# ylsung/vl-merging

Hardware: AMD Instinct MI355X
Metric: VL samples/sec (fwd+bwd) base_vl 384^2 at 1/2/4/8 GPUs; merge GB/s vs HBM peak (higher is better)
Workload: dtype bf16

## Files before the change

include/vlm_hip.h:

```cpp
#ifndef VLM_HIP_H
#define VLM_HIP_H
#include <stddef.h>
#include <stdint.h>

#ifdef __cplusplus
extern "C" {
#endif

#define VLM_OK 0
#define VLM_ERR_ARG (-1)
#define VLM_ERR_LAUNCH (-2)
#define VLM_ERR_WORKSPACE (-3)
#define VLM_ERR_UNSUPPORTED (-4)

#define VLM_ABI_VERSION 11
int vlm_abi_version(void);
int vlm_device_cus(void);
int vlm_set_cu_budget(int cus);
int vlm_debug_occupy(int workgroups, int threads, int lds_bytes, int microseconds, void* stream);

#define VLM_MERGE_LERP 0
#define VLM_MERGE_TASKVEC 1
#define VLM_MERGE_MEAN 2
#define VLM_MERGE_MAX_SRC 4
// ... 392 lines not shown
                  int ldc, int c_is_f32, const vlm_epilogue_t* epi, void* stream);
int vlm_gemm_bf16_live(int ta, int tb, int M, int N, int K, const void* A, int lda, const void* B, int ldb, void* C,
                       int ldc, int c_is_f32, const vlm_epilogue_t* epi, const float* row_live, void* stream);
#define VLM_GEMM_MAX_GROUPS 4
typedef struct {
  int32_t row0, rows;
  const void* B;
  int32_t ldb;
  int32_t reserved;
  const float* bias;
  float* col_sum;
  float* col_sum_ws;
} vlm_gemm_group_t;
int vlm_gemm_bf16_grouped(int n_groups, const vlm_gemm_group_t* groups, int N, int K, const void* A, int lda, void* C,
                          int ldc, int c_is_f32, const vlm_epilogue_t* epi, void* stream);
typedef struct {
  int32_t row0, rows;
  float* C;
  int32_t accumulate;
  int32_t reserved;
} vlm_wgrad_group_t;
int vlm_gemm_wgrad_grouped(int n_groups, const vlm_wgrad_group_t* groups, int M, int N, const void* A, int lda,
                           const void* B, int ldb, int ldc, float* splitk_ws, uint64_t splitk_ws_bytes, void* stream);
typedef struct {
  const void* dy;
  int32_t ld_dy, M;
  const void* x;
  int32_t ld_x, N;
  float* dW;
  int32_t ldc, accumulate;
} vlm_wgrad_problem_t;
int vlm_gemm_wgrad_batch(int n, const vlm_wgrad_problem_t* problems, int T, float* splitk_ws, uint64_t splitk_ws_bytes,
                         void* stream);
int vlm_gemm_set_big_tile_mode(int mode);

int vlm_layernorm_fwd(const float* x, int ldx, int M, int D, const float* gamma, const float* beta, float eps,
                      void* y, int ldy, int y_is_f32, float* stats, void* stream);
#define VLM_ROW_WS_BYTES(D) ((size_t)1536 * 2 * (size_t)(D) * sizeof(float))
int vlm_layernorm_bwd(const void* dy, int lddy, int dy_is_f32, const float* x, int ldx, const float* stats,
                      const float* gamma, int M, int D, const float* dres, int lddres, float* dx, int lddx,
                      float* dgamma, float* dbeta, float* workspace, size_t workspace_bytes, int* deferred_blocks,
                      void* stream);
typedef struct {
  const void* y;
  int32_t ldy;
  const float* gamma;
  const float* row_scale;
  void* dy;
  int32_t lddy;
  float* dgamma;
  float* dbias;
  float* workspace;
  size_t workspace_bytes;
} vlm_layerscale_t;
int vlm_layernorm_bwd_scale(const void* dy, int lddy, int dy_is_f32, const float* x, int ldx, const float* stats,
                            const float* gamma, int M, int D, const float* dres, int lddres, float* dx, int lddx,
                            float* dgamma, float* dbeta, float* workspace, size_t workspace_bytes,
                            const vlm_layerscale_t* scale, int* deferred_blocks, void* stream);
#define VLM_MAX_FOLD_JOBS 16
typedef struct {
  const float* partials;
  int32_t nblocks;
  int32_t D;
  float* out0;
  float* out1;
} vlm_fold_job_t;
// ... 188 lines not shown
```

vl-merging_amd/_lib.py:

```python
import ctypes
import os

_HERE = os.path.dirname(os.path.abspath(__file__))
LIB_PATH = os.environ.get("VLM_LIB_PATH") or os.path.join(_HERE, "lib", "libvlm_hip.so")
_lib = None

c_void_p = ctypes.c_void_p
c_int = ctypes.c_int
c_float = ctypes.c_float
c_size_t = ctypes.c_size_t
c_u64 = ctypes.c_uint64

MERGE_LERP, MERGE_TASKVEC, MERGE_MEAN = 0, 1, 2
MERGE_MAX_SRC = 4


class MergeJob(ctypes.Structure):
    _fields_ = [
        ("dst", c_void_p),
        ("base", c_void_p),
        ("src", c_void_p * MERGE_MAX_SRC),
        ("ratio", c_float * MERGE_MAX_SRC),
        ("n_src", ctypes.c_int32),
        ("mode", ctypes.c_int32),
# ... 370 lines not shown
    "vlm_band_plan_bytes": (c_size_t, [c_int, c_u64]),
    "vlm_band_plan_upload": (c_int, [ctypes.POINTER(BandJob), c_int, c_void_p, c_size_t, c_void_p]),
    "vlm_band_run": (c_int, [c_void_p, c_void_p]),
    "vlm_della_plan_bytes": (c_size_t, [c_int, c_u64]),
    "vlm_della_plan_upload": (c_int, [ctypes.POINTER(DellaJob), c_int, c_void_p, c_size_t, c_void_p]),
    "vlm_della_run": (c_int, [c_void_p, c_void_p]),
    "vlm_pairstats_plan_bytes": (c_size_t, [c_int, c_u64]),
    "vlm_pairstats_plan_upload": (c_int, [ctypes.POINTER(PairStatsJob), c_int, c_void_p, c_size_t, c_void_p]),
    "vlm_pairstats_run": (c_int, [c_void_p, c_void_p]),
    "vlm_stock_plan_bytes": (c_size_t, [c_int, c_u64]),
    "vlm_stock_plan_upload": (c_int, [ctypes.POINTER(StockJob), c_int, c_void_p, c_size_t, c_void_p]),
    "vlm_stock_run": (c_int, [c_void_p, c_void_p]),
    "vlm_sce_plan_bytes": (c_size_t, [c_int, c_u64]),
    "vlm_sce_plan_upload": (c_int, [ctypes.POINTER(SceJob), c_int, c_void_p, c_size_t, c_void_p]),
    "vlm_sce_run": (c_int, [c_void_p, c_void_p]),
    "vlm_sphere_plan_bytes": (c_size_t, [c_int, c_u64]),
    "vlm_sphere_plan_upload": (c_int, [ctypes.POINTER(SphereJob), c_int, c_void_p, c_size_t, c_void_p]),
    "vlm_sphere_run": (c_int, [c_void_p, c_void_p]),
    "vlm_tall_plan_bytes": (c_size_t, [c_int, c_u64]),
    "vlm_tall_plan_upload": (c_int, [ctypes.POINTER(TallJob), c_int, c_void_p, c_size_t, c_void_p]),
    "vlm_tall_run": (c_int, [c_void_p, c_void_p]),
    "vlm_emr_plan_bytes": (c_size_t, [c_int, c_u64]),
    "vlm_emr_plan_upload": (c_int, [ctypes.POINTER(EmrJob), c_int, c_void_p, c_size_t, c_void_p]),
    "vlm_emr_run": (c_int, [c_void_p, c_void_p]),
    "vlm_gemm_bf16": (c_int, [c_int, c_int, c_int, c_int, c_int, c_void_p, c_int, c_void_p, c_int, c_void_p, c_int,
                              c_int, ctypes.POINTER(Epilogue), c_void_p]),
    "vlm_gemm_bf16_live": (c_int, [c_int, c_int, c_int, c_int, c_int, c_void_p, c_int, c_void_p, c_int, c_void_p, c_int,
                                   c_int, ctypes.POINTER(Epilogue), c_void_p, c_void_p]),
    "vlm_gemm_bf16_grouped": (c_int, [c_int, ctypes.POINTER(GemmGroup), c_int, c_int, c_void_p, c_int, c_void_p, c_int, c_int,
                                      ctypes.POINTER(Epilogue), c_void_p]),
    "vlm_gemm_wgrad_grouped": (c_int, [c_int, ctypes.POINTER(WgradGroup), c_int, c_int, c_void_p, c_int, c_void_p, c_int, c_int,
                                       c_void_p, c_u64, c_void_p]),
    "vlm_gemm_wgrad_batch": (c_int, [c_int, ctypes.POINTER(WgradProblem), c_int, c_void_p, c_u64, c_void_p]),
    "vlm_attention_fwd": (c_int, [ctypes.POINTER(AttnDesc), c_void_p, c_int, c_void_p, c_void_p]),
    "vlm_attention_bwd_ws_floats": (c_size_t, [ctypes.POINTER(AttnDesc), c_int]),
    "vlm_attention_qkeep_served": (c_int, [ctypes.POINTER(AttnDesc), c_int]),
    "vlm_attention_bwd": (c_int, [ctypes.POINTER(AttnDesc), c_void_p, c_int, c_void_p, c_int, c_void_p, c_void_p, c_size_t,
                                  c_void_p, c_int, c_void_p, c_void_p, c_void_p]),
    "vlm_attention_bwd_live": (c_int, [ctypes.POINTER(AttnDesc), c_void_p, c_int, c_void_p, c_int, c_void_p, c_void_p, c_size_t,
                                       c_void_p, c_int, c_void_p, c_void_p, c_void_p, c_void_p]),
    "vlm_layernorm_fwd": (c_int, [c_void_p, c_int, c_int, c_int, c_void_p, c_void_p, c_float, c_void_p, c_int, c_int,
                                  c_void_p, c_void_p]),
    "vlm_layernorm_bwd": (c_int, [c_void_p, c_int, c_int, c_void_p, c_int, c_void_p, c_void_p, c_int, c_int, c_void_p,
                                  c_int, c_void_p, c_int, c_void_p, c_void_p, c_void_p, c_size_t,
                                  ctypes.POINTER(c_int), c_void_p]),
    "vlm_layernorm_bwd_scale": (c_int, [c_void_p, c_int, c_int, c_void_p, c_int, c_void_p, c_void_p, c_int, c_int, c_void_p,
                                        c_int, c_void_p, c_int, c_void_p, c_void_p, c_void_p, c_size_t,
                                        ctypes.POINTER(LayerScale), ctypes.POINTER(c_int), c_void_p]),
    "vlm_layerscale_bwd": (c_int, [c_void_p, c_int, c_void_p, c_int, c_void_p, c_void_p, c_int, c_int, c_void_p, c_int,
                                   c_void_p, c_void_p, c_void_p, c_size_t, ctypes.POINTER(c_int), c_void_p]),
    "vlm_colreduce_batch": (c_int, [ctypes.POINTER(FoldJob), c_int, c_void_p]),
    "vlm_gemm_set_big_tile_mode": (c_int, [c_int]),
    "vlm_colsum_bf16": (c_int, [c_void_p, c_int, c_int, c_int, c_void_p, c_void_p]),
    "vlm_adamw_step": (c_int, [c_void_p, c_void_p, c_void_p, c_void_p, c_void_p, c_u64, c_float, c_float, c_float,
                               c_float, c_float, c_float, c_float, c_int, c_void_p]),
    "vlm_accumulate_f32_f64": (c_int, [c_void_p, c_void_p, c_u64, c_void_p]),
    "vlm_gram_f64": (c_int, [c_void_p, c_int, c_int, c_int, c_int, c_void_p, c_void_p]),
    "vlm_gemm_f64": (c_int, [c_int, c_int, c_int, c_int, c_int, ctypes.c_double, c_void_p, c_int, c_int, c_void_p, c_int,
                             ctypes.c_double, c_void_p, c_int, c_void_p]),
    "vlm_scale_gram_f64": (c_int, [c_void_p, c_void_p, c_int, ctypes.c_double, c_int, c_void_p]),
    "vlm_cholesky_f64": (c_int, [c_void_p, c_int, c_void_p, c_void_p]),
    "vlm_solve_spd_right_f64": (c_int, [c_void_p, c_int, c_void_p, c_int, c_int, c_void_p]),
    "vlm_gemm_f64_batched": (c_int, [c_int, c_int, c_int, c_int, c_int, ctypes.c_double, ctypes.POINTER(c_void_p), c_int, c_int,
                                     ctypes.POINTER(c_void_p), c_int, ctypes.c_double, ctypes.POINTER(c_void_p), c_int, c_int, c_void_p]),
    "vlm_cholesky_f64_batched": (c_int, [ctypes.POINTER(c_void_p), c_int, c_int, c_void_p, c_void_p]),
    "vlm_solve_spd_right_f64_batched": (c_int, [ctypes.POINTER(c_void_p), c_int, ctypes.POINTER(c_void_p), c_int, c_int, c_int, c_void_p]),
# ... 103 lines not shown
```

vl-merging_amd/csrc/gemm.hip:

```cpp
#include "vlm_common.h"
#include "vlm_diag.h"
#include "wgrad_plan.h"
#include <atomic>

#define GEMM_BM 128
#define GEMM_BN 128
#define GEMM_BK 64
#define GEMM_THREADS 256
#define GEMM_TILE_BYTES (GEMM_BM * GEMM_BK * 2)

typedef __attribute__((address_space(3))) s16x4 lds_s16x4;

__device__ __forceinline__ float gelu_cdf(float x, float& ez2) {
  const float t = __builtin_amdgcn_rcpf(fmaf(0.3275911f * 0.70710678118654752440f, fabsf(x), 1.0f));
  ez2 = __builtin_amdgcn_exp2f((x * x) * (-0.5f * 1.4426950408889634f));
  float poly = fmaf(t, 0.5f * 1.061405429f, 0.5f * -1.453152027f);
  poly = fmaf(t, poly, 0.5f * 1.421413741f);
  poly = fmaf(t, poly, 0.5f * -0.284496736f);
  poly = fmaf(t, poly, 0.5f * 0.254829592f);
  const float e = fmaf(-(poly * t), ez2, 0.5f);
  return 0.5f + copysignf(e, x);
}
__device__ __forceinline__ float gelu_erf(float x) {
  float ez2;
// ... 910 lines not shown
  asm volatile("s_waitcnt lgkmcnt(0)" ::: "memory");
  __builtin_amdgcn_s_barrier();
  BIG_READ(fa0, fb0, sA0, sB0)
  GEMM_STAMP(1)

  int kt = 0;
  for (; kt < nk - 4; kt += 2) {
    BIG_STEP(kt + 0, 1, 1, 1, fa0, fb0, fa1, fb1, ra0, rb0, sA0, sB0, sA1, sB1)
    BIG_STEP(kt + 1, 1, 1, 1, fa1, fb1, fa0, fb0, ra1, rb1, sA1, sB1, sA0, sB0)
  }
#define BIG_TAIL_STEPS()                                                               \
  BIG_STEP(kt + 0, 0, 1, 1, fa0, fb0, fa1, fb1, ra0, rb0, sA0, sB0, sA1, sB1)          \
  BIG_STEP(kt + 1, 0, 1, 1, fa1, fb1, fa0, fb0, ra1, rb1, sA1, sB1, sA0, sB0)          \
  BIG_STEP(kt + 2, 0, 0, 1, fa0, fb0, fa1, fb1, ra0, rb0, sA0, sB0, sA1, sB1)          \
  BIG_STEP(kt + 3, 0, 0, 0, fa1, fb1, fa0, fb0, ra1, rb1, sA1, sB1, sA0, sB0)
  if constexpr (DEEP) {
    BIG_TAIL_STEPS()
    GEMM_STAMP(2)
    big_epilogue_t<OUT_F32, RES, AUX> ep(p, wl, mw0, nw0, lane);
    float* ws_row = (p.epi.col_sum_ws && mw0 + 128 <= (uint32_t)p.M) ? p.epi.col_sum_ws + ((size_t)(tm_ws * 2 + wm) * 2) * p.N : nullptr;
    BIG_EPILOGUE_LOOP_DEEP(AHEAD)
    ep.finish(lane, ws_row);
  } else {
    EPIL_SETUP()
    BIG_TAIL_STEPS()
    GEMM_STAMP(2)
    float* ws_row = (p.epi.col_sum_ws && mw0 + 128 <= (uint32_t)p.M) ? p.epi.col_sum_ws + ((size_t)(tm_ws * 2 + wm) * 2) * p.N : nullptr;
    BIG_EPILOGUE_LOOP()
    ep.finish(lane, ws_row);
  }
  GEMM_STAMP_END()
}

template <bool GROUPED = false>
__global__ __launch_bounds__(GEMM_THREADS, 1) void vlm_gemm_bigT_kernel(const gemm_params_t p) {
  __shared__ __attribute__((aligned(1024))) unsigned char sA0[BIG_OP_BYTES], sA1[BIG_OP_BYTES], sB0[BIG_OP_BYTES], sB1[BIG_OP_BYTES];
  __shared__ __attribute__((aligned(16))) unsigned char epl[4 * EPIL_WAVE_BYTES];
  const int tid = threadIdx.x;
  const int lane = tid & 63;
  const int wave = __builtin_amdgcn_readfirstlane(tid >> 6);
  const int wm = wave >> 1, wn = wave & 1;
  uint32_t ntile = p.tiles_m * p.tiles_n, tiles_n = (uint32_t)p.tiles_n;
  const uint32_t q8 = gridDim.x >> 3, r8 = gridDim.x & 7, xcd = blockIdx.x & 7;
  uint32_t item = (xcd < r8 ? xcd * (q8 + 1) : r8 * (q8 + 1) + (xcd - r8) * q8) + (blockIdx.x >> 3);
  uint32_t k_base = 0, k_end = (uint32_t)p.K, ws_base = 0;
  int nk = p.ksteps_per_split;
  const void *A = p.A, *B = p.B;
  uint32_t lda = (uint32_t)p.lda, ldb = (uint32_t)p.ldb;
  int M = p.M, N = p.N;
  if constexpr (GROUPED) {
    int g = 0;
#pragma unroll
    for (int i = 1; i < VLM_GEMM_MAX_GROUPS; ++i)
      if (i < p.n_groups && item >= (uint32_t)p.grpT[i].item0) g = i;
    const gemmT_group_t G = p.grpT[g];
    item -= (uint32_t)G.item0;
    k_base = (uint32_t)G.row0;
    k_end = (uint32_t)G.row_end;
    nk = G.kps;
    ws_base = G.ws_base;
    A = G.A; B = G.B;
    lda = (uint32_t)G.lda; ldb = (uint32_t)G.ldb;
    M = G.M; N = G.N;
    ntile = (uint32_t)G.ntile; tiles_n = (uint32_t)G.tiles_n;
  }
  const uint32_t split = item / ntile, tile = item - split * ntile;
  const uint32_t tm = tile / tiles_n, tn = tile - tm * tiles_n;
  const uint32_t m0 = tm * BIG_BM, n0 = tn * BIG_BN;
  const uint32_t k_first = k_base + split * (uint32_t)nk * BIG_BK;
  const __amdgpu_buffer_rsrc_t ra =
      __builtin_amdgcn_make_buffer_rsrc(const_cast<void*>(A), 0, (int)((uint64_t)k_end * lda * 2), 0x00020000);
  const __amdgpu_buffer_rsrc_t rb =
      __builtin_amdgcn_make_buffer_rsrc(const_cast<void*>(B), 0, (int)((uint64_t)k_end * ldb * 2), 0x00020000);

  uint32_t offa[4], offb[4], wr_off[4];
#pragma unroll
  for (int u = 0; u < 4; ++u) {
    const uint32_t row = 2 * (wave + 4 * u) + (lane >> 5), c16 = lane & 31;
    offa[u] = ((k_first + row) * lda + m0 + c16 * 8) * 2;
    offb[u] = ((k_first + row) * ldb + n0 + c16 * 8) * 2;
    wr_off[u] = row * 512 + (((c16 >> 1) ^ ((row & 3) | (((row >> 3) & 1) << 2))) << 5) + (c16 & 1) * 16;
  }
  uint32_t rda[8], rdb[8];
  {
// ... 48 lines not shown
    BIG_MFMA(FCA, FCB)                                                                   \
    _Pragma("unroll") for (int g = 0; g < 32; ++g) {                                     \
      __builtin_amdgcn_sched_group_barrier(0x008, 1, 0);                                 \
      __builtin_amdgcn_sched_group_barrier(0x100, 1, 0);                                 \
    }                                                                                    \
    _Pragma("unroll") for (int g = 0; g < 8; ++g) {                                      \
      __builtin_amdgcn_sched_group_barrier(0x008, 2, 0);                                 \
      __builtin_amdgcn_sched_group_barrier(0x200, 1, 0);                                 \
      __builtin_amdgcn_sched_group_barrier(0x008, 2, 0);                                 \
      __builtin_amdgcn_sched_group_barrier(0x020, 1, 0);                                 \
    }                                                                                    \
    __builtin_amdgcn_sched_barrier(0);                                                   \
  }
  BIGT_GLOAD(ra0, rb0, 0)
  BIGT_GLOAD(ra1, rb1, 1)
  BIGT_LWRITE(ra0, rb0, sA0, sB0)
  BIGT_GLOAD(ra0, rb0, 2)
  BIGT_LWRITE(ra1, rb1, sA1, sB1)
  BIGT_GLOAD(ra1, rb1, 3)
  asm volatile("s_waitcnt lgkmcnt(0)" ::: "memory");
  __builtin_amdgcn_s_barrier();
  BIGT_READ(fa0, fb0, sA0, sB0)
  int kt = 0;
  for (; kt < nk - 4; kt += 2) {
    BIGT_STEP(kt + 0, 1, 1, 1, fa0, fb0, fa1, fb1, ra0, rb0, sA0, sB0, sA1, sB1)
    BIGT_STEP(kt + 1, 1, 1, 1, fa1, fb1, fa0, fb0, ra1, rb1, sA1, sB1, sA0, sB0)
  }
  BIGT_STEP(kt + 0, 0, 1, 1, fa0, fb0, fa1, fb1, ra0, rb0, sA0, sB0, sA1, sB1)
  BIGT_STEP(kt + 1, 0, 1, 1, fa1, fb1, fa0, fb0, ra1, rb1, sA1, sB1, sA0, sB0)
  BIGT_STEP(kt + 2, 0, 0, 1, fa0, fb0, fa1, fb1, ra0, rb0, sA0, sB0, sA1, sB1)
  BIGT_STEP(kt + 3, 0, 0, 0, fa1, fb1, fa0, fb0, ra1, rb1, sA1, sB1, sA0, sB0)

  gemm_params_t pl = p;
  pl.C = reinterpret_cast<float*>(p.C) + ws_base + (size_t)split * M * N;
  pl.M = M;
  pl.N = N;
  pl.ldc = N;
  const uint32_t mw0 = m0 + wm * 128, nw0 = n0 + wn * 128;
  unsigned char* const wl = epl + wave * EPIL_WAVE_BYTES;
  big_epilogue_t<true, false, 0, 128, 0, true> ep(pl, wl, mw0, nw0, lane);
  epil_in_t inA, inB;
  ep.load_inputs(inA, 0);
  BIG_EPILOGUE_LOOP()
}

__global__ __launch_bounds__(256) void splitk_reduce_kernel(const float* __restrict__ ws, int splits, int M, int N, float* __restrict__ C,
                                                            int ldc, int accumulate) {
  const size_t i = (size_t)blockIdx.x * 256 + threadIdx.x, per = (size_t)M * N / 4;
  if (i >= per) return;
  const size_t e = i * 4, m = e / N, n = e - m * N;
  f32x4 t = accumulate ? *reinterpret_cast<const f32x4*>(C + m * ldc + n) : (f32x4){0.f, 0.f, 0.f, 0.f};
  for (int s = 0; s < splits; ++s) t += *reinterpret_cast<const f32x4*>(ws + (size_t)s * M * N + e);
  *reinterpret_cast<f32x4*>(C + m * ldc + n) = t;
}

struct splitk_groups_t {
  float* C[VLM_GEMM_MAX_GROUPS];
  int M[VLM_GEMM_MAX_GROUPS], N[VLM_GEMM_MAX_GROUPS], ldc[VLM_GEMM_MAX_GROUPS];
  uint32_t ws_base[VLM_GEMM_MAX_GROUPS];
  int splits[VLM_GEMM_MAX_GROUPS], accumulate[VLM_GEMM_MAX_GROUPS];
};
__global__ __launch_bounds__(256) void splitk_reduce_grouped_kernel(const float* __restrict__ ws, const splitk_groups_t g) {
  const int gi = blockIdx.y;
  const int N = g.N[gi], ldc = g.ldc[gi];
  const size_t i = (size_t)blockIdx.x * 256 + threadIdx.x, mn = (size_t)g.M[gi] * N;
  if (i >= mn / 4) return;
  float* const C = g.C[gi];
  const float* const w = ws + g.ws_base[gi];
  const size_t e = i * 4, m = e / N, n = e - m * N;
  f32x4 t = g.accumulate[gi] ? *reinterpret_cast<const f32x4*>(C + m * ldc + n) : (f32x4){0.f, 0.f, 0.f, 0.f};
  for (int s = 0; s < g.splits[gi]; ++s) t += *reinterpret_cast<const f32x4*>(w + (size_t)s * mn + e);
  *reinterpret_cast<f32x4*>(C + m * ldc + n) = t;
}

static int plan_cus() {
  const int cus = vlm_device_cus();
// ... 269 lines not shown
  p.n_groups = n;
  splitk_groups_t rg{};
  size_t per = 0;
  for (int g = 0; g < n; ++g) {
    const wgradT_problem_t& P = pr[g];
    const wgrad_plan_group_t& G = plan.g[g];
    p.grpT[g] = gemmT_group_t{P.A, P.B, P.lda, P.ldb, P.M, P.N, P.N / BIG_BN, in[g].tiles, P.row0, P.row_end, G.item0, G.kps,
                              (uint32_t)G.ws_base};
    rg.C[g] = P.C; rg.M[g] = P.M; rg.N[g] = P.N; rg.ldc[g] = P.ldc;
    rg.ws_base[g] = (uint32_t)G.ws_base; rg.splits[g] = G.splits; rg.accumulate[g] = P.accumulate;
    if ((size_t)P.M * P.N / 4 > per) per = (size_t)P.M * P.N / 4;
  }
  hipLaunchKernelGGL(vlm_gemm_bigT_kernel<true>, dim3(plan.items), dim3(GEMM_THREADS), 0, s, p);
  VLM_CHECK_LAUNCH();
  hipLaunchKernelGGL(splitk_reduce_grouped_kernel, dim3((unsigned)((per + 255) / 256), n), dim3(256), 0, s,
                     reinterpret_cast<const float*>(splitk_ws), rg);
  VLM_CHECK_LAUNCH();
  return VLM_OK;
}

extern "C" int vlm_gemm_wgrad_batch(int n, const vlm_wgrad_problem_t* problems, int T, float* splitk_ws, uint64_t splitk_ws_bytes,
                                    void* stream) {
  if (n < 1 || n > VLM_GEMM_MAX_GROUPS || !problems || T < 1) return VLM_ERR_ARG;
  wgradT_problem_t pr[VLM_GEMM_MAX_GROUPS];
  for (int i = 0; i < n; ++i) {
    const vlm_wgrad_problem_t& P = problems[i];
    if (!P.dy || !P.x || !P.dW || P.M < 1 || P.N < 1) return VLM_ERR_ARG;
    pr[i] = wgradT_problem_t{P.dy, P.x, P.ld_dy, P.ld_x, P.M, P.N, 0, T, P.dW, P.ldc, P.accumulate};
  }
  if (gemm_big_mode() <= 0) return 1;
  return launch_gemm_bigT_grouped(n, pr, splitk_ws, splitk_ws_bytes, (hipStream_t)stream);
}

extern "C" int vlm_gemm_wgrad_grouped(int n_groups, const vlm_wgrad_group_t* groups, int M, int N, const void* A, int lda,
                                      const void* B, int ldb, int ldc, float* splitk_ws, uint64_t splitk_ws_bytes, void* stream) {
  if (n_groups < 1 || n_groups > VLM_GEMM_MAX_GROUPS || !groups || M < 0 || N < 0) return VLM_ERR_ARG;
  int prev_end = 0;
  for (int g = 0; g < n_groups; ++g) {
    if (groups[g].row0 < prev_end || groups[g].rows < 0 || !groups[g].C) return VLM_ERR_ARG;
    prev_end = groups[g].row0 + groups[g].rows;
  }
  if (M == 0 || N == 0) return VLM_OK;
  if (!A || !B || (lda & 7) || (ldb & 7) || ((uintptr_t)A & 15) || ((uintptr_t)B & 15)) return VLM_ERR_ARG;
  hipStream_t s = (hipStream_t)stream;
  for (int g = 0; g < n_groups; ++g)
    if (groups[g].rows == 0 && !groups[g].accumulate &&
        hipMemset2DAsync(groups[g].C, (size_t)ldc * 4, 0, (size_t)N * 4, M, s) != hipSuccess)
      return VLM_ERR_LAUNCH;
  const int K_total = prev_end;
  if (gemm_big_mode() > 0 && (uint64_t)K_total * lda * 2 < (1ull << 31) && (uint64_t)K_total * ldb * 2 < (1ull << 31)) {
    wgradT_problem_t pr[VLM_GEMM_MAX_GROUPS];
    int live = 0;
    for (int g = 0; g < n_groups; ++g) {
      const vlm_wgrad_group_t& G = groups[g];
      if (G.rows > 0) pr[live++] = wgradT_problem_t{A, B, lda, ldb, M, N, G.row0, G.row0 + G.rows, G.C, ldc, G.accumulate};
    }
    if (live == 0) return VLM_OK;
    const int rc = launch_gemm_bigT_grouped(live, pr, splitk_ws, splitk_ws_bytes, s);
    if (rc <= 0) return rc;
  }
  for (int g = 0; g < n_groups; ++g) {
    const vlm_wgrad_group_t& G = groups[g];
    if (G.rows == 0) continue;
    vlm_epilogue_t e{};
    e.alpha = 1.0f;
    e.accumulate = G.accumulate;
// ... 11 lines not shown
```

vl-merging_amd/csrc/wgrad_plan.h:

```cpp
#pragma once
#include <stddef.h>
#include <stdint.h>

#define WGRAD_PLAN_MAX_GROUPS 4
#define WGRAD_PLAN_MIN_STEPS 16

struct wgrad_plan_in_t {
  int tiles;
  int ksteps;
  uint64_t mn;
};

struct wgrad_plan_group_t {
  int kps, splits;
  int item0;
  int slice0;
  uint64_t ws_base;
};

struct wgrad_plan_t {
  wgrad_plan_group_t g[WGRAD_PLAN_MAX_GROUPS];
  int items;
  int slices;
  uint64_t ws_floats;
// ... 7 lines not shown
    if (in[g].tiles == 0 || in[g].ksteps == 0) continue;
    tiles += in[g].tiles;
    work += (long)in[g].ksteps * in[g].tiles;
  }
  if (tiles == 0 || tiles > cus) return 1;
  long target = (work + cus - 1) / cus;
  if (target < WGRAD_PLAN_MIN_STEPS) target = WGRAD_PLAN_MIN_STEPS;
  for (;; target += 2) {
    long items = 0;
    for (int g = 0; g < n; ++g)
      if (in[g].tiles > 0 && in[g].ksteps > 0) items += ((in[g].ksteps + target - 1) / target) * in[g].tiles;
    if (items <= cus) break;
  }
  out->items = out->slices = 0;
  out->ws_floats = 0;
  for (int g = 0; g < n; ++g) {
    wgrad_plan_group_t& G = out->g[g];
    G = wgrad_plan_group_t{0, 0, out->items, out->slices, out->ws_floats};
    if (in[g].tiles == 0 || in[g].ksteps == 0) continue;
    const int nk = in[g].ksteps;
    int splits = (int)((nk + target - 1) / target);
    int kps = (nk + splits - 1) / splits;
    kps += kps & 1;
    if (kps < 4) kps = 4;
    splits = (nk + kps - 1) / kps;
    G.kps = kps;
    G.splits = splits;
    out->items += splits * in[g].tiles;
    out->slices += splits;
    out->ws_floats += (uint64_t)splits * in[g].mn;
  }
  return out->ws_floats > ws_floats ? 1 : 0;
}
```

vl-merging_amd/engine.py:

```python
import itertools
import math
import os
import weakref
from typing import List, Optional

import torch

from . import _lib as L
from . import ops

BF16, F32 = torch.bfloat16, torch.float32
ALIGN = 64


def _touch_hook(p):
    p._vlm_flat.touched.add(p._vlm_name)


def touch(*params):
    for p in params:
        if p is not None:
            f = getattr(p, "_vlm_flat", None)
            if f is not None:
                f.touched.add(p._vlm_name)
# ... 131 lines not shown
        layers = sorted(pend) if layer is None else ([layer] if layer in pend else [])
        if not layers:
            return
        jobs = [j for i in layers for j in self._ls_jobs.get(i, ())]
        side = wgrad_stream()
        if side is None:
            ops.layerscale_finish(jobs)
        else:
            side.wait_stream(torch.cuda.current_stream())
            with torch.cuda.stream(side):
                ops.layerscale_finish(jobs)
            if not _WGRAD["pending"]:
                torch.cuda.current_stream().wait_stream(side)
        for i in layers:
            pend.discard(i)

    def zero_grad(self):
        self.flat_g.zero_()
        if getattr(self, "ls_pending", None) or getattr(self, "_ls_armed", False):
            for jobs in getattr(self, "_ls_jobs", {}).values():
                for j in jobs:
                    j["raw_w"].zero_()
                    if j["raw_b"] is not None:
                        j["raw_b"].zero_()
            self.ls_pending.clear()
            self._ls_armed = False

    def slice_of(self, names):
        lo = min(self.offsets[n][0] for n in names)
        hi = max(self.offsets[n][0] + self.extent[n] for n in names)
        return lo, hi


_WGRAD = {"stream": None, "enabled": os.environ.get("VLM_WGRAD_STREAM", "1") != "0", "pending": False}


def wgrad_stream():
    if not _WGRAD["enabled"]:
        return None
    if _WGRAD["stream"] is None:
        _WGRAD["stream"] = torch.cuda.Stream()
    return _WGRAD["stream"]


def sync_wgrad():
    if _WGRAD["stream"] is not None:
        torch.cuda.current_stream().wait_stream(_WGRAD["stream"])
    _WGRAD["pending"] = False


def _arm_wgrad_join():
    if not _WGRAD["pending"]:
        _WGRAD["pending"] = True
        torch.autograd.Variable._execution_engine.queue_callback(sync_wgrad)


class _Side:

    def __init__(self, *tensors):
        self.s = wgrad_stream()
        self.tensors = tensors
        self.ctx = None

    def __enter__(self):
        if self.s is None:
            return self
        self.s.wait_stream(torch.cuda.current_stream())
# ... 508 lines not shown
        plan, pc = ctx.plan, ctx.pc
        x, st1, ln1, qkv, o, lse, y1, x1, st2, ln2, h, a, y2, rs1, rs2, bias_t, ok = ctx.saved_tensors
        kr = ctx.kr
        rs1 = rs1 if rs1.numel() else None
        rs2 = rs2 if rs2.numel() else None
        live_all = _live(rs1, plan, pc)
        if kr is not None:
            rs1, rs2 = kr.take(rs1), kr.take(rs2)
        live1, live2 = _live(rs1, plan, pc), _live(rs2, plan, pc)
        bias_t = bias_t if ctx.has_bias else None
        M_all, D = x.shape
        M = x1.shape[0]
        dev = x.device
        H = pc.H
        Fdim = h.shape[1]
        if ctx.kr_out is not None:
            dx2 = ctx.kr_out.put(dx2.contiguous(), M_all, F32)
        dx2 = dx2.contiguous()
        g1, g2 = plan.gamma1, plan.gamma2
        folded = ctx.folded
        if folded:
            y1 = y2 = None
            flat = plan.ranges[0][2].projw._vlm_flat
            _arm_layerscale_finish(flat)
        wg = (lambda w: w._vlm_raw) if folded else (lambda w: w.grad)
        touch(g1, g2)
        for _, _, e in plan.ranges:
            _touch_expert(e)
        dy2 = torch.empty(M, D, device=dev, dtype=BF16)
        dy1 = torch.empty(M, D, device=dev, dtype=BF16)
        dh = torch.empty(M, Fdim, device=dev, dtype=BF16)
        dln = torch.empty(M, D, device=dev, dtype=BF16)
        dx1 = torch.empty(M, D, device=dev, dtype=F32)
        fold = ops.FoldBatch(dev, D)
        rg_all = plan.ranges
        rg = kr.ranges(rg_all) if kr is not None else rg_all
        if kr is None:
            ok, do_all = o, torch.empty(M_all, D, device=dev, dtype=BF16)
            do = do_all
        elif kr.span is not None:
            ok, do_all = kr.take(o), torch.empty(M_all, D, device=dev, dtype=BF16)
            do = kr.take(do_all)
        else:
            do_all, do = None, torch.empty(M, D, device=dev, dtype=BF16)
        for r0, r1, e in rg:
            rr = slice(r0, r1)
            if folded:
                ops.layerscale_bwd(dx2[rr], None, None, rs2[rr] if rs2 is not None else None, dy2[rr], None, _rb(e.fc2b), fold=fold)
            else:
                ops.layerscale_bwd(dx2[rr], y2[rr], g2, rs2[rr] if rs2 is not None else None, dy2[rr], g2.grad, e.fc2b.grad,
                                   fold=fold)
        _gemm_rows(dy2, [(r0, r1, wT16(e.fc2w), None, e.fc1b.grad) for r0, r1, e in rg], dh, act=L.ACT_MUL_AUX, aux=h,
                   col_sum_fold=fold, row_live=live2)
        tail3 = [(D, Fdim), (Fdim, D), (D, D)]
        batch = wgrad_stream() is not None and len(rg) == 1 and ops.wgrad_batch_serves(
            rg[0][1] - rg[0][0], tail3 + ([(3 * D, D)] if kr is None else []))
        if not batch:
            with _Side(dy2, a, dh, ln2):
                _wgrad_rows(dy2, a, [(r0, r1, wg(e.fc2w)) for r0, r1, e in rg])
                _wgrad_rows(dh, ln2, [(r0, r1, e.fc1w.grad) for r0, r1, e in rg])
        _gemm_rows(dh, [(r0, r1, wT16(e.fc1w), None, None) for r0, r1, e in rg], dln, row_live=live2)
        for r0, r1, e in rg:
            rr = slice(r0, r1)
            _ln2_bwd_scale1(dln[rr], x1[rr], st2[rr], e, dx1[rr], dx2[rr], y1[rr] if y1 is not None else None, g1,
                            rs1[rr] if rs1 is not None else None, dy1[rr], fold)
        _gemm_rows(dy1, [(r0, r1, wT16(e.projw), None, None) for r0, r1, e in rg], do, row_live=live1)
        if not batch:
            with _Side(dy1, ok):
                _wgrad_rows(dy1, ok, [(r0, r1, wg(e.projw)) for r0, r1, e in rg])
        if do_all is None:
            do_all = kr.put(do, M_all, BF16)
        dqkv = torch.empty(M_all, 3 * D, device=dev, dtype=BF16)
        dln1 = torch.empty(M_all, D, device=dev, dtype=BF16)
        rp = pc.relpos
        qb_grads, vb_grads, fused_qv = _segment_bias_grads(rg_all, pc.seq)
        dbias_acc = rp.holder.get("dbias_t") if rp is not None else None
        if kr is not None and dbias_acc is None:
            dbias_acc = torch.zeros_like(bias_t)
        ops.attention_bwd(qkv, o, do_all, lse, dqkv, pc.seq, H, bias_t=bias_t, head_row0=plan.layer * H,
                          rel_index=rp.index if rp is not None else None,
                          rel_index_t=rp.index_t if rp is not None else None, keep0=pc.keep0, keep1=pc.keep1,
                          mode=plan.mode, dbias_t=dbias_acc,
                          dq_colsum=qb_grads, dv_colsum=vb_grads,
                          bias_dense=rp.dense_for(pc.seq, plan.mode) if rp is not None else None, row_live=live_all,
                          q_keep=kr.q if kr is not None else None)
        dx = torch.empty(M_all, D, device=dev, dtype=F32)
        for r0, r1, e in rg_all:
            if e.qb is not None and not fused_qv:
                ops.colsum(dqkv[r0:r1, :D], e.qb.grad)
                ops.colsum(dqkv[r0:r1, 2 * D:], e.vb.grad)
        if batch:
            (r0, r1, e), = rg
            rr = slice(r0, r1)
            with _Side(dy2, a, dh, ln2, dy1, ok, dqkv, ln1):
                tail = [(dy2[rr], a[rr], wg(e.fc2w)), (dh[rr], ln2[rr], e.fc1w.grad), (dy1[rr], ok[rr], wg(e.projw))]
                if kr is None:
                    ops.gemm_wgrad_batch(tail + [(dqkv[rr], ln1[rr], e.qkvw.grad)])
                else:
                    ops.gemm_wgrad_batch(tail)
                    _wgrad_rows(dqkv, ln1, [(q0, q1, eq.qkvw.grad) for q0, q1, eq in rg_all])
        else:
            with _Side(dqkv, ln1):
                _wgrad_rows(dqkv, ln1, [(r0, r1, e.qkvw.grad) for r0, r1, e in rg_all])
        _gemm_rows(dqkv, [(r0, r1, wT16(e.qkvw), None, None) for r0, r1, e in rg_all], dln1, row_live=live_all)
        if kr is not None and kr.span is None:
            dx1 = kr.put(dx1, M_all, F32)
        for r0, r1, e in rg_all:
            for p0, p1, at in ([(r0, r1, r0)] if kr is None or kr.span is None else kr.pieces(r0, r1)):
                rr = slice(p0, p1)
                ops.layernorm_bwd(dln1[rr], x[rr], st1[rr], e.n1w, dx[rr], dres=dx1[at:at + p1 - p0] if at is not None else None,
                                  dgamma=e.n1w.grad, dbeta=e.n1b.grad, fold=fold)
        fold.flush()
        if folded:
            flat.ls_pending.add(plan.layer)
        if ctx.hook is not None:
            ctx.hook(plan.layer)
        dbias = None
        if bias_t is not None and ctx.needs_input_grad[1] and rp is not None and not rp.holder.get("routed"):
            rp.holder["routed"] = True
            dbias = _zero_scalar(dev).expand_as(bias_t)
        return dx, dbias, None, None, None, None, None, None


def run_block(x, plan: BlockPlan, pc: PassCtx, training: bool, hook=None, keep=None):
    bias_t = pc.relpos.bias_t if pc.relpos is not None else None
    if keep is not None and KeepRows.of(pc.seq, keep) is None:
        raise L.VlmError("run_block: keep must name whole segments or first rows, got %r" % (keep,))
    recorded = torch.is_grad_enabled() and (x.requires_grad or (bias_t is not None and bias_t.requires_grad))
    return _BlockFn.apply(x, bias_t, plan, pc, training, hook, keep, recorded)


def _kernel_rows(t, dtypes=(BF16, F32), row_align=1, ptr_align=1, layout=True):
    if not (torch.is_tensor(t) and t.is_cuda and t.dtype in dtypes):
        return False
    return not layout or (t.dim() == 2 and t.stride(1) == 1 and t.stride(0) % row_align == 0 and t.data_ptr() % ptr_align == 0)


def _rows2d(g, D, dtypes=(BF16, F32), contiguous=False):
    g2 = g.reshape(-1, D)
    if g2.dtype not in dtypes:
        g2 = g2.float()
    return g2.contiguous() if contiguous or g2.stride(1) != 1 else g2


class _LinearFn(torch.autograd.Function):
# ... 445 lines not shown
```

vl-merging_amd/ops.py:

```python
import ctypes

import torch

from . import _lib as L

BF16 = torch.bfloat16
F32 = torch.float32


def _ld(t):
    if t.dim() != 2 or t.stride(1) != 1:
        raise L.VlmError("expected a 2-D tensor with unit inner stride, got shape %s strides %s"
                         % (tuple(t.shape), t.stride()))
    return t.stride(0) if t.shape[0] > 1 else max(t.stride(0), t.shape[1])


_SCRATCH = {}


def _scratch(kind, floats, device):
    key = (kind, device.index, torch.cuda.current_stream().cuda_stream)
    ws = _SCRATCH.get(key)
    if ws is None or ws.numel() < floats:
        ws = _SCRATCH[key] = torch.empty(floats, device=device, dtype=F32)
# ... 107 lines not shown
                                           int(out.dtype == F32), ctypes.byref(e), L.stream_ptr())
    L.check(rc, "vlm_gemm_bf16_grouped")
    return out


def gemm_wgrad_grouped(dy, x, groups, accumulate=True):
    L.require_cuda(dy, x)
    if dy.dtype != BF16 or x.dtype != BF16 or dy.shape[0] != x.shape[0]:
        raise L.VlmError("gemm_wgrad_grouped: bf16 dy [tokens, M] and x [tokens, N]")
    M, N = dy.shape[1], x.shape[1]
    arr = (L.WgradGroup * len(groups))()
    prev, ldc = 0, None
    for g, (r0, r1, dW) in zip(arr, groups):
        L.require_cuda(dW)
        if dW.dtype != F32 or tuple(dW.shape) != (M, N) or r0 < prev or r1 < r0 or r1 > dy.shape[0]:
            raise L.VlmError("gemm_wgrad_grouped: group (%d, %d) gradient %s for M=%d N=%d" % (r0, r1, tuple(dW.shape), M, N))
        if ldc is not None and _ld(dW) != ldc:
            raise L.VlmError("gemm_wgrad_grouped: the groups' gradients must share one leading dimension")
        ldc = _ld(dW)
        prev = r1
        g.row0, g.rows, g.C, g.accumulate = r0, r1 - r0, dW.data_ptr(), int(bool(accumulate))
    ws = _scratch("splitk", SPLITK_WS_BYTES // 4, dy.device)
    rc = L.get_lib().vlm_gemm_wgrad_grouped(len(groups), arr, M, N, L.ptr(dy), _ld(dy), L.ptr(x), _ld(x), ldc, L.ptr(ws),
                                            ws.numel() * 4, L.stream_ptr())
    L.check(rc, "vlm_gemm_wgrad_grouped")


def wgrad_batch_serves(T, shapes):
    cus = L.get_lib().vlm_device_cus()
    return (T >= 2048 and 1 <= len(shapes) <= L.GEMM_MAX_GROUPS and all(N % 256 == 0 for _, N in shapes)
            and sum(-(-M // 256) * (N // 256) for M, N in shapes) <= (cus if cus > 0 else 256))


def gemm_wgrad_batch(problems, accumulate=True):
    n = len(problems)
    if n < 1 or n > L.GEMM_MAX_GROUPS:
        raise L.VlmError("gemm_wgrad_batch: 1..%d problems" % L.GEMM_MAX_GROUPS)
    acc = [bool(accumulate)] * n if isinstance(accumulate, (bool, int)) else [bool(f) for f in accumulate]
    if len(acc) != n:
        raise L.VlmError("gemm_wgrad_batch: one accumulate flag, or one per problem")
    T = problems[0][0].shape[0]
    arr = (L.WgradProblem * n)()
    for g, (dy, x, dW), f in zip(arr, problems, acc):
        L.require_cuda(dy, x, dW)
        if dy.dtype != BF16 or x.dtype != BF16 or dW.dtype != F32 or dy.dim() != 2 or x.dim() != 2 or dW.dim() != 2:
            raise L.VlmError("gemm_wgrad_batch: bf16 dy [T, M] and x [T, N], f32 dW [M, N]")
        if dy.shape[0] != T or x.shape[0] != T or tuple(dW.shape) != (dy.shape[1], x.shape[1]):
            raise L.VlmError("gemm_wgrad_batch: dy %s, x %s, dW %s over T=%d rows" % (tuple(dy.shape), tuple(x.shape),
                                                                                      tuple(dW.shape), T))
        g.dy, g.ld_dy, g.M = dy.data_ptr(), _ld(dy), dy.shape[1]
        g.x, g.ld_x, g.N = x.data_ptr(), _ld(x), x.shape[1]
        g.dW, g.ldc, g.accumulate = dW.data_ptr(), _ld(dW), int(f)
    rc = 1
    if T >= 2048:
        ws = _scratch("splitk", SPLITK_WS_BYTES // 4, problems[0][0].device)
        rc = L.get_lib().vlm_gemm_wgrad_batch(n, arr, T, L.ptr(ws), ws.numel() * 4, L.stream_ptr())
    if rc == 1:
        for (dy, x, dW), f in zip(problems, acc):
            gemm(dy, x, dW, ta=True, tb=True, accumulate=f)
        return
    L.check(rc, "vlm_gemm_wgrad_batch")


def layernorm_fwd(x, gamma, beta, eps, out, stats=None):
    L.require_cuda(x, gamma, beta, out, stats)
    M, D = x.shape
    rc = L.get_lib().vlm_layernorm_fwd(L.ptr(x), _ld(x), M, D, L.ptr(gamma), L.ptr(beta), eps, L.ptr(out), _ld(out),
                                       int(out.dtype == F32), L.ptr(stats), L.stream_ptr())
    L.check(rc, "vlm_layernorm_fwd")
    return out


def _row_ws_floats(D):
    return 1536 * 2 * max(D, 1024)


class FoldBatch:

    MAX = 16

    def __init__(self, device, D=1024):
        self.region = _row_ws_floats(D)
        self.ws = _scratch("fold", self.MAX * self.region, device)
        self.jobs = []
        self.taken = 0

    def next_region(self):
        return self.next_regions(1)[0]

    def next_regions(self, n):
        if self.taken + n > self.MAX:
            self.flush()
        i = self.taken
        self.taken += n
        return [self.ws[(i + k) * self.region:(i + k + 1) * self.region] for k in range(n)]

    def add(self, region, nblocks, D, out0, out1):
        if nblocks > 0:
            self.jobs.append((region, nblocks, D, out0, out1))

    def flush(self):
        self.taken = 0
        if not self.jobs:
            return
        arr = (L.FoldJob * len(self.jobs))()
        for a, (region, nblocks, D, out0, out1) in zip(arr, self.jobs):
            a.partials, a.nblocks, a.D = region.data_ptr(), nblocks, D
            a.out0 = out0.data_ptr() if out0 is not None else None
            a.out1 = out1.data_ptr() if out1 is not None else None
        L.check(L.get_lib().vlm_colreduce_batch(arr, len(self.jobs), L.stream_ptr()), "vlm_colreduce_batch")
        self.jobs = []


def _row_bwd(name, fold, device, D, head, pairs, sc=None):
    ws = (fold.next_regions(len(pairs)) if fold is not None
          else [_scratch("row%d" % k, _row_ws_floats(D), device) for k in range(len(pairs))])
# ... 901 lines not shown
```

Before: 369.8.

## Add whole-K weight-gradient kernel without split-K and move fold flush to side stream

New measurement: 372.9, median of 6. Within noise of the previous version (+0.8%).

```diff
diff --git a/include/vlm_hip.h b/include/vlm_hip.h
--- a/include/vlm_hip.h
+++ b/include/vlm_hip.h
@@ -448,6 +448,7 @@
 } vlm_wgrad_problem_t;
 int vlm_gemm_wgrad_batch(int n, const vlm_wgrad_problem_t* problems, int T, float* splitk_ws, uint64_t splitk_ws_bytes,
                          void* stream);
+int vlm_gemm_wgrad_whole(int n, const vlm_wgrad_problem_t* problems, int T, void* stream);
 int vlm_gemm_set_big_tile_mode(int mode);
 
 int vlm_layernorm_fwd(const float* x, int ldx, int M, int D, const float* gamma, const float* beta, float eps,
diff --git a/vl-merging_amd/_lib.py b/vl-merging_amd/_lib.py
--- a/vl-merging_amd/_lib.py
+++ b/vl-merging_amd/_lib.py
@@ -426,6 +426,7 @@
     "vlm_gemm_wgrad_grouped": (c_int, [c_int, ctypes.POINTER(WgradGroup), c_int, c_int, c_void_p, c_int, c_void_p, c_int, c_int,
                                        c_void_p, c_u64, c_void_p]),
     "vlm_gemm_wgrad_batch": (c_int, [c_int, ctypes.POINTER(WgradProblem), c_int, c_void_p, c_u64, c_void_p]),
+    "vlm_gemm_wgrad_whole": (c_int, [c_int, ctypes.POINTER(WgradProblem), c_int, c_void_p]),
     "vlm_attention_fwd": (c_int, [ctypes.POINTER(AttnDesc), c_void_p, c_int, c_void_p, c_void_p]),
     "vlm_attention_bwd_ws_floats": (c_size_t, [ctypes.POINTER(AttnDesc), c_int]),
     "vlm_attention_qkeep_served": (c_int, [ctypes.POINTER(AttnDesc), c_int]),
diff --git a/vl-merging_amd/csrc/gemm.hip b/vl-merging_amd/csrc/gemm.hip
--- a/vl-merging_amd/csrc/gemm.hip
+++ b/vl-merging_amd/csrc/gemm.hip
@@ -966,8 +966,13 @@
   GEMM_STAMP_END()
 }
 
-template <bool GROUPED = false>
-__global__ __launch_bounds__(GEMM_THREADS, 1) void vlm_gemm_bigT_kernel(const gemm_params_t p) {
+struct wgrad_whole_t {
+  float* C[VLM_GEMM_MAX_GROUPS];
+  int ldc[VLM_GEMM_MAX_GROUPS], accumulate[VLM_GEMM_MAX_GROUPS];
+};
+
+template <bool GROUPED, bool WHOLE>
+__device__ __forceinline__ void gemm_bigT_body(const gemm_params_t& p, const wgrad_whole_t* whole) {
   __shared__ __attribute__((aligned(1024))) unsigned char sA0[BIG_OP_BYTES], sA1[BIG_OP_BYTES], sB0[BIG_OP_BYTES], sB1[BIG_OP_BYTES];
   __shared__ __attribute__((aligned(16))) unsigned char epl[4 * EPIL_WAVE_BYTES];
   const int tid = threadIdx.x;
@@ -982,8 +987,8 @@
   const void *A = p.A, *B = p.B;
   uint32_t lda = (uint32_t)p.lda, ldb = (uint32_t)p.ldb;
   int M = p.M, N = p.N;
+  int g = 0;
   if constexpr (GROUPED) {
-    int g = 0;
 #pragma unroll
     for (int i = 1; i < VLM_GEMM_MAX_GROUPS; ++i)
       if (i < p.n_groups && item >= (uint32_t)p.grpT[i].item0) g = i;
@@ -1098,16 +1103,36 @@
   BIGT_STEP(kt + 3, 0, 0, 0, fa1, fb1, fa0, fb0, ra1, rb1, sA1, sB1, sA0, sB0)
 
   gemm_params_t pl = p;
-  pl.C = reinterpret_cast<float*>(p.C) + ws_base + (size_t)split * M * N;
   pl.M = M;
   pl.N = N;
-  pl.ldc = N;
   const uint32_t mw0 = m0 + wm * 128, nw0 = n0 + wn * 128;
   unsigned char* const wl = epl + wave * EPIL_WAVE_BYTES;
-  big_epilogue_t<true, false, 0, 128, 0, true> ep(pl, wl, mw0, nw0, lane);
-  epil_in_t inA, inB;
-  ep.load_inputs(inA, 0);
-  BIG_EPILOGUE_LOOP()
+  if constexpr (WHOLE) {
+    pl.C = whole->C[g];
+    pl.ldc = whole->ldc[g];
+    pl.epi.residual = whole->accumulate[g] ? whole->C[g] : nullptr;
+    pl.epi.ld_res = whole->ldc[g];
+    big_epilogue_t<true, true, 0, 128, 0> ep(pl, wl, mw0, nw0, lane);
+    epil_in_t inA, inB;
+    ep.load_inputs(inA, 0);
+    BIG_EPILOGUE_LOOP()
+  } else {
+    pl.C = reinterpret_cast<float*>(p.C) + ws_base + (size_t)split * M * N;
+    pl.ldc = N;
+    big_epilogue_t<true, false, 0, 128, 0, true> ep(pl, wl, mw0, nw0, lane);
+    epil_in_t inA, inB;
+    ep.load_inputs(inA, 0);
+    BIG_EPILOGUE_LOOP()
+  }
+}
+
+template <bool GROUPED = false>
+__global__ __launch_bounds__(GEMM_THREADS, 1) void vlm_gemm_bigT_kernel(const gemm_params_t p) {
+  gemm_bigT_body<GROUPED, false>(p, nullptr);
+}
+
+__global__ __launch_bounds__(GEMM_THREADS, 1) void vlm_wgrad_whole_kernel(const gemm_params_t p, const wgrad_whole_t whole) {
+  gemm_bigT_body<true, true>(p, &whole);
 }
 
 __global__ __launch_bounds__(256) void splitk_reduce_kernel(const float* __restrict__ ws, int splits, int M, int N, float* __restrict__ C,
@@ -1443,6 +1468,51 @@
   return launch_gemm_bigT_grouped(n, pr, splitk_ws, splitk_ws_bytes, (hipStream_t)stream);
 }
 
+extern "C" int vlm_gemm_wgrad_whole(int n, const vlm_wgrad_problem_t* problems, int T, void* stream) {
+  if (n < 1 || n > VLM_GEMM_MAX_GROUPS || !problems || T < 1) return VLM_ERR_ARG;
+  for (int i = 0; i < n; ++i) {
+    const vlm_wgrad_problem_t& P = problems[i];
+    if (!P.dy || !P.x || !P.dW || P.M < 1 || P.N < 1) return VLM_ERR_ARG;
+  }
+  if (gemm_big_mode() <= 0) return 1;
+  wgrad_plan_in_t in[VLM_GEMM_MAX_GROUPS];
+  for (int g = 0; g < n; ++g) {
+    const vlm_wgrad_problem_t& P = problems[g];
+    if ((P.N % BIG_BN) || (P.ldc % 4) || P.ldc < P.N || ((uintptr_t)P.dW & 15) || ((uintptr_t)P.dy & 15) || ((uintptr_t)P.x & 15) ||
+        (P.ld_dy & 7) || (P.ld_x & 7) || P.ld_dy < P.M || P.ld_x < P.N)
+      return 1;
+    if ((uint64_t)P.M * P.N * 4 >= (1ull << 31) || (uint64_t)P.M * P.ldc * 4 >= (1ull << 31) ||
+        (uint64_t)T * P.ld_dy * 2 >= (1ull << 31) || (uint64_t)T * P.ld_x * 2 >= (1ull << 31))
+      return 1;
+    const uint64_t m_up = (uint64_t)(P.M + BIG_BM - 1) / BIG_BM * BIG_BM, t_up = (uint64_t)T + 6 * BIG_BK;
+    if (m_up * P.ldc * 4 >= (1ull << 32) || t_up * P.ld_dy * 2 >= (1ull << 32) || t_up * P.ld_x * 2 >= (1ull << 32)) return 1;
+    in[g] = wgrad_plan_in_t{((P.M + BIG_BM - 1) / BIG_BM) * (P.N / BIG_BN), (T + BIG_BK - 1) / BIG_BK, (uint64_t)P.M * P.N};
+  }
+  wgrad_plan_t plan;
+  if (wgrad_plan_whole(n, in, plan_cus(), &plan)) return 1;
+  gemm_params_t p;
+  p.A = nullptr; p.B = nullptr; p.C = nullptr;
+  p.M = 0; p.N = 0; p.K = 0;
+  p.lda = 0; p.ldb = 0; p.ldc = 0;
+  p.epi = vlm_epilogue_t{};
+  p.epi.alpha = 1.0f;
+  p.epi.reserved = 1;
+  p.tiles_m = 0; p.tiles_n = 0;
+  p.group_m = 1;
+  p.splits = 1;
+  p.ksteps_per_split = 0;
+  p.n_groups = n;
+  wgrad_whole_t w{};
+  for (int g = 0; g < n; ++g) {
+    const vlm_wgrad_problem_t& P = problems[g];
+    p.grpT[g] = gemmT_group_t{P.dy, P.x, P.ld_dy, P.ld_x, P.M, P.N, P.N / BIG_BN, in[g].tiles, 0, T, plan.g[g].item0, plan.g[g].kps, 0u};
+    w.C[g] = P.dW; w.ldc[g] = P.ldc; w.accumulate[g] = P.accumulate;
+  }
+  hipLaunchKernelGGL(vlm_wgrad_whole_kernel, dim3(plan.items), dim3(GEMM_THREADS), 0, (hipStream_t)stream, p, w);
+  VLM_CHECK_LAUNCH();
+  return VLM_OK;
+}
+
 extern "C" int vlm_gemm_wgrad_grouped(int n_groups, const vlm_wgrad_group_t* groups, int M, int N, const void* A, int lda,
                                       const void* B, int ldb, int ldc, float* splitk_ws, uint64_t splitk_ws_bytes, void* stream) {
   if (n_groups < 1 || n_groups > VLM_GEMM_MAX_GROUPS || !groups || M < 0 || N < 0) return VLM_ERR_ARG;
diff --git a/vl-merging_amd/csrc/wgrad_plan.h b/vl-merging_amd/csrc/wgrad_plan.h
--- a/vl-merging_amd/csrc/wgrad_plan.h
+++ b/vl-merging_amd/csrc/wgrad_plan.h
@@ -63,3 +63,27 @@
   }
   return out->ws_floats > ws_floats ? 1 : 0;
 }
+
+static inline int wgrad_plan_whole(int n, const wgrad_plan_in_t* in, int cus, wgrad_plan_t* out) {
+  if (n < 1 || n > WGRAD_PLAN_MAX_GROUPS || cus < 1) return 1;
+  long tiles = 0;
+  for (int g = 0; g < n; ++g) {
+    if (in[g].tiles < 0 || in[g].ksteps < 0) return 1;
+    if (in[g].tiles > 0 && in[g].ksteps > 0) tiles += in[g].tiles;
+  }
+  if (tiles == 0 || tiles > cus) return 1;
+  out->items = out->slices = 0;
+  out->ws_floats = 0;
+  for (int g = 0; g < n; ++g) {
+    wgrad_plan_group_t& G = out->g[g];
+    G = wgrad_plan_group_t{0, 0, out->items, out->slices, 0};
+    if (in[g].tiles == 0 || in[g].ksteps == 0) continue;
+    int kps = in[g].ksteps + (in[g].ksteps & 1);
+    if (kps < 4) kps = 4;
+    G.kps = kps;
+    G.splits = 1;
+    out->items += in[g].tiles;
+    out->slices += 1;
+  }
+  return 0;
+}
diff --git a/vl-merging_amd/engine.py b/vl-merging_amd/engine.py
--- a/vl-merging_amd/engine.py
+++ b/vl-merging_amd/engine.py
@@ -187,7 +187,8 @@
         return lo, hi
 
 
-_WGRAD = {"stream": None, "enabled": os.environ.get("VLM_WGRAD_STREAM", "1") != "0", "pending": False}
+_WGRAD = {"stream": None, "enabled": os.environ.get("VLM_WGRAD_STREAM", "1") != "0", "pending": False, "whole": True,
+          "fold_side": True, "fold_turn": 0, "fold_done": [None, None]}
 
 
 def wgrad_stream():
@@ -762,7 +763,14 @@
         dh = torch.empty(M, Fdim, device=dev, dtype=BF16)
         dln = torch.empty(M, D, device=dev, dtype=BF16)
         dx1 = torch.empty(M, D, device=dev, dtype=F32)
-        fold = ops.FoldBatch(dev, D)
+        fold_side = wgrad_stream() is not None and _WGRAD["fold_side"]
+        half = None
+        if fold_side:
+            half = _WGRAD["fold_turn"]
+            _WGRAD["fold_turn"] = half ^ 1
+            if _WGRAD["fold_done"][half] is not None:
+                torch.cuda.current_stream().wait_event(_WGRAD["fold_done"][half])
+        fold = ops.FoldBatch(dev, D, half=half)
         rg_all = plan.ranges
         rg = kr.ranges(rg_all) if kr is not None else rg_all
         if kr is None:
@@ -785,6 +793,7 @@
         tail3 = [(D, Fdim), (Fdim, D), (D, D)]
         batch = wgrad_stream() is not None and len(rg) == 1 and ops.wgrad_batch_serves(
             rg[0][1] - rg[0][0], tail3 + ([(3 * D, D)] if kr is None else []))
+        wgrad_batch = ops.gemm_wgrad_whole if _WGRAD["whole"] and not (_WGRAD.get("tail_sliced") and plan.layer == 0) else ops.gemm_wgrad_batch
         if not batch:
             with _Side(dy2, a, dh, ln2):
                 _wgrad_rows(dy2, a, [(r0, r1, wg(e.fc2w)) for r0, r1, e in rg])
@@ -825,10 +834,14 @@
             with _Side(dy2, a, dh, ln2, dy1, ok, dqkv, ln1):
                 tail = [(dy2[rr], a[rr], wg(e.fc2w)), (dh[rr], ln2[rr], e.fc1w.grad), (dy1[rr], ok[rr], wg(e.projw))]
                 if kr is None:
-                    ops.gemm_wgrad_batch(tail + [(dqkv[rr], ln1[rr], e.qkvw.grad)])
+                    wgrad_batch(tail + [(dqkv[rr], ln1[rr], e.qkvw.grad)])
                 else:
-                    ops.gemm_wgrad_batch(tail)
-                    _wgrad_rows(dqkv, ln1, [(q0, q1, eq.qkvw.grad) for q0, q1, eq in rg_all])
+                    wgrad_batch(tail)
+                    if _WGRAD["whole"] and len(rg_all) == 1:
+                        (q0, q1, eq), = rg_all
+                        wgrad_batch([(dqkv[q0:q1], ln1[q0:q1], eq.qkvw.grad)])
+                    else:
+                        _wgrad_rows(dqkv, ln1, [(q0, q1, eq.qkvw.grad) for q0, q1, eq in rg_all])
         else:
             with _Side(dqkv, ln1):
                 _wgrad_rows(dqkv, ln1, [(r0, r1, e.qkvw.grad) for r0, r1, e in rg_all])
@@ -840,7 +853,13 @@
                 rr = slice(p0, p1)
                 ops.layernorm_bwd(dln1[rr], x[rr], st1[rr], e.n1w, dx[rr], dres=dx1[at:at + p1 - p0] if at is not None else None,
                                   dgamma=e.n1w.grad, dbeta=e.n1b.grad, fold=fold)
-        fold.flush()
+        if fold_side:
+            with _Side(fold.ws) as side:
+                fold.flush()
+                done = _WGRAD["fold_done"][half] = _WGRAD["fold_done"][half] or torch.cuda.Event()
+                done.record(side.s)
+        else:
+            fold.flush()
         if folded:
             flat.ls_pending.add(plan.layer)
         if ctx.hook is not None:
diff --git a/vl-merging_amd/ops.py b/vl-merging_amd/ops.py
--- a/vl-merging_amd/ops.py
+++ b/vl-merging_amd/ops.py
@@ -163,34 +163,48 @@
             and sum(-(-M // 256) * (N // 256) for M, N in shapes) <= (cus if cus > 0 else 256))
 
 
-def gemm_wgrad_batch(problems, accumulate=True):
+def _wgrad_problems(name, problems, accumulate):
     n = len(problems)
     if n < 1 or n > L.GEMM_MAX_GROUPS:
-        raise L.VlmError("gemm_wgrad_batch: 1..%d problems" % L.GEMM_MAX_GROUPS)
+        raise L.VlmError("%s: 1..%d problems" % (name, L.GEMM_MAX_GROUPS))
     acc = [bool(accumulate)] * n if isinstance(accumulate, (bool, int)) else [bool(f) for f in accumulate]
     if len(acc) != n:
-        raise L.VlmError("gemm_wgrad_batch: one accumulate flag, or one per problem")
+        raise L.VlmError("%s: one accumulate flag, or one per problem" % name)
     T = problems[0][0].shape[0]
     arr = (L.WgradProblem * n)()
     for g, (dy, x, dW), f in zip(arr, problems, acc):
         L.require_cuda(dy, x, dW)
         if dy.dtype != BF16 or x.dtype != BF16 or dW.dtype != F32 or dy.dim() != 2 or x.dim() != 2 or dW.dim() != 2:
-            raise L.VlmError("gemm_wgrad_batch: bf16 dy [T, M] and x [T, N], f32 dW [M, N]")
+            raise L.VlmError("%s: bf16 dy [T, M] and x [T, N], f32 dW [M, N]" % name)
         if dy.shape[0] != T or x.shape[0] != T or tuple(dW.shape) != (dy.shape[1], x.shape[1]):
-            raise L.VlmError("gemm_wgrad_batch: dy %s, x %s, dW %s over T=%d rows" % (tuple(dy.shape), tuple(x.shape),
-                                                                                      tuple(dW.shape), T))
+            raise L.VlmError("%s: dy %s, x %s, dW %s over T=%d rows" % (name, tuple(dy.shape), tuple(x.shape), tuple(dW.shape), T))
         g.dy, g.ld_dy, g.M = dy.data_ptr(), _ld(dy), dy.shape[1]
         g.x, g.ld_x, g.N = x.data_ptr(), _ld(x), x.shape[1]
         g.dW, g.ldc, g.accumulate = dW.data_ptr(), _ld(dW), int(f)
+    return arr, T, acc
+
+
+def gemm_wgrad_batch(problems, accumulate=True):
+    arr, T, acc = _wgrad_problems("gemm_wgrad_batch", problems, accumulate)
     rc = 1
     if T >= 2048:
         ws = _scratch("splitk", SPLITK_WS_BYTES // 4, problems[0][0].device)
-        rc = L.get_lib().vlm_gemm_wgrad_batch(n, arr, T, L.ptr(ws), ws.numel() * 4, L.stream_ptr())
+        rc = L.get_lib().vlm_gemm_wgrad_batch(len(problems), arr, T, L.ptr(ws), ws.numel() * 4, L.stream_ptr())
     if rc == 1:
         for (dy, x, dW), f in zip(problems, acc):
             gemm(dy, x, dW, ta=True, tb=True, accumulate=f)
         return
     L.check(rc, "vlm_gemm_wgrad_batch")
+
+
+def gemm_wgrad_whole(problems, accumulate=True):
+    arr, T, acc = _wgrad_problems("gemm_wgrad_whole", problems, accumulate)
+    rc = L.get_lib().vlm_gemm_wgrad_whole(len(problems), arr, T, L.stream_ptr())
+    if rc == 1:
+        for (dy, x, dW), f in zip(problems, acc):
+            gemm(dy, x, dW, ta=True, tb=True, accumulate=f)
+        return
+    L.check(rc, "vlm_gemm_wgrad_whole")
 
 
 def layernorm_fwd(x, gamma, beta, eps, out, stats=None):
@@ -210,9 +224,9 @@
 
     MAX = 16
 
-    def __init__(self, device, D=1024):
+    def __init__(self, device, D=1024, half=None):
         self.region = _row_ws_floats(D)
-        self.ws = _scratch("fold", self.MAX * self.region, device)
+        self.ws = _scratch("fold" if half is None else "fold%d" % half, self.MAX * self.region, device)
         self.jobs = []
         self.taken = 0
 
```
